# migoox/genome-downsampler

Hardware: AMD Instinct MI355X
Metric: Mreads/s selected at target coverage M=100 (higher is better)
Workload: dtype u32

## Files before the change

### genome-downsampler_amd/csrc/kernels/pass_major.inc.hip

```cpp
static constexpr int kPmPass = 8192;
__host__ __device__ inline uint32_t pm_stride_of(uint32_t n_ranges) { return (uint32_t)kPmPass + 64u * n_ranges; }
static constexpr int kPmThreads = 512;
static constexpr int kPmWaves = kPmThreads / 64;
static constexpr int kPmPassesPerWg = 4;
static constexpr size_t kPmSortLds = ((size_t)kPmPass + kPmWaves * 256 + 2 * 256 + 16 + 2 * kPmPassesPerWg * 256 + kPmWaves * 3 * 128) * sizeof(uint32_t);
static constexpr uint32_t kPmExcPerWave = 128;

#ifndef QMCP_PM_MIN_WAVES
#define QMCP_PM_MIN_WAVES 4
#endif
__global__ __launch_bounds__(kPmThreads, QMCP_PM_MIN_WAVES) void k_pm_prepare_sort(
    const uint32_t* __restrict__ starts, const uint32_t* __restrict__ ends, uint32_t n,
    const uint64_t* __restrict__ contig_read_off, const uint64_t* __restrict__ contig_pos_off, uint32_t n_contigs,
    const uint32_t* __restrict__ vbase ,
    uint32_t shift, uint32_t stride ,
    uint16_t* __restrict__ keys16, uint16_t* __restrict__ idx16,
    uint32_t* __restrict__ cnt_tab, uint32_t* __restrict__ lst_tab, uint32_t pitch ,
    uint32_t* __restrict__ stats, unsigned long long* __restrict__ zero_mask,
    uint32_t ell_reg, uint32_t* __restrict__ exc, uint32_t exc_cap, uint32_t* __restrict__ exc_cnt) {
    extern __shared__ uint32_t s_pm[];
    uint32_t* s_stage = s_pm;
    uint32_t* s_cnt = s_stage + kPmPass;
    uint32_t* s_gbase = s_cnt + kPmWaves * 256;
    uint32_t* s_pbase = s_gbase + 256;
    uint32_t* s_wave = s_pbase + 256;
    uint32_t* s_tabc = s_wave + 16;
    uint32_t* s_tabl = s_tabc + kPmPassesPerWg * 256;
    uint32_t* s_exc = s_tabl + kPmPassesPerWg * 256;
    const int lane = threadIdx.x & 63, w = threadIdx.x >> 6;
    uint32_t mn = 0xFFFFFFFFu, mx = 0, bad = 0;
    auto contig_of = [&](uint32_t i) {
        uint32_t lo = 0, hi = n_contigs;
        while (hi - lo > 1) {
            const uint32_t mid = (lo + hi) >> 1;
            if (contig_read_off[mid] <= i) lo = mid; else hi = mid;
        }
        return lo;
    };
    for (int g = 0; g < kPmPassesPerWg; ++g) {
        const uint32_t P = blockIdx.x * kPmPassesPerWg + g;
        const uint64_t base64 = (uint64_t)P * kPmPass;
        if (base64 >= n) {
            if (threadIdx.x < 256) { s_tabc[g * 256 + threadIdx.x] = 0; s_tabl[g * 256 + threadIdx.x] = 0; }
            if (ell_reg != 0u && lane == 0 && P < pitch) exc_cnt[P * kPmWaves + w] = 0;
            continue;
        }
        const uint32_t base = (uint32_t)base64;
        const uint32_t count = min((uint32_t)kPmPass, n - base);
        const uint32_t wbase = base + w * (kSortItems * 64);
        Rec rec[kSortItems];
#pragma unroll
        for (int k = 0; k < kSortItems; ++k) {
            const uint32_t i = min(wbase + k * 64 + lane, n - 1);
            rec[k].key = starts[i];
            rec[k].val = ends[i];
        }
        for (int i = threadIdx.x; i < kPmWaves * 256; i += kPmThreads) s_cnt[i] = 0;
        if (zero_mask && threadIdx.x < 128 && P * 128u + threadIdx.x < (n + 63u) / 64u) zero_mask[P * 128u + threadIdx.x] = 0ull;
        const uint32_t c_first = n_contigs > 1 ? contig_of(base) : 0u;
        const uint32_t c_last = n_contigs > 1 ? contig_of(base + count - 1) : 0u;
        uint32_t match_bits;
        {
            const uint32_t len_last = (uint32_t)(contig_pos_off[c_last + 1] - contig_pos_off[c_last]);
            const uint32_t d_lo = (vbase[c_first] >> shift) & 255u;
            const uint32_t d_hi = ((vbase[c_last] + (len_last ? len_last - 1u : 0u)) >> shift) & 255u;
            match_bits = d_hi >= d_lo ? 32u - (uint32_t)__builtin_clz((d_hi - d_lo) | 1u) : 8u;
            if (d_hi == d_lo) match_bits = 0;
        }
        uint32_t skip = 0;
        uint32_t filled = 0;
        typedef __attribute__((address_space(3))) uint32_t LdsWord;
        LdsWord* const mine = (LdsWord*)(s_exc + w * (3 * kPmExcPerWave));
        auto put_aside = [&, mine](int k, bool isx, uint32_t gs, uint32_t ge, uint32_t i) {
            const uint64_t m = __ballot(isx);
            if (m != 0ull) {
                const uint32_t slot = filled + __builtin_amdgcn_mbcnt_hi((uint32_t)(m >> 32), __builtin_amdgcn_mbcnt_lo((uint32_t)m, 0u));
                if (isx) {
                    skip |= 1u << k;
                    if (slot < kPmExcPerWave) { mine[3u * slot] = gs; mine[3u * slot + 1u] = ge; mine[3u * slot + 2u] = i; }
                    else nu_overflow_put(exc, exc_cap, stats, gs, ge, i);
                }
                filled += (uint32_t)__popcll(m);
            }
        };
        if (c_first == c_last) {
            const uint32_t p0 = (uint32_t)contig_pos_off[c_first];
            const uint32_t len = (uint32_t)contig_pos_off[c_first + 1] - p0;
            const uint32_t v0 = vbase[c_first];
            const uint32_t last = len ? len - 1u : 0u;
#pragma unroll
            for (int k = 0; k < kSortItems; ++k) {
                const uint32_t i = wbase + k * 64 + lane;
                const uint32_t s = rec[k].key, e = rec[k].val;
                bool isx = false;
                if (i < n) {
                    bad |= (s > e || e >= len) ? 1u : 0u;
                    const uint32_t span = e - s + 1;
                    mn = min(mn, span);
                    mx = max(mx, span);
                    isx = span != ell_reg;
                }
                rec[k].key = v0 + min(s, last);
                if (ell_reg != 0u) put_aside(k, isx, p0 + min(s, last), p0 + min(e, last), i);
            }
        } else {
#pragma unroll
            for (int k = 0; k < kSortItems; ++k) {
                const uint32_t i = wbase + k * 64 + lane;
                bool isx = false;
                uint32_t gs = 0, ge = 0;
                if (i < n) {
                    const uint32_t cc = contig_of(i);
                    const uint32_t p0 = (uint32_t)contig_pos_off[cc];
                    const uint32_t len = (uint32_t)contig_pos_off[cc + 1] - p0;
                    const uint32_t s = rec[k].key, e = rec[k].val;
                    bad |= (s > e || e >= len) ? 1u : 0u;
                    const uint32_t span = e - s + 1;
                    mn = min(mn, span);
                    mx = max(mx, span);
                    rec[k].key = vbase[cc] + min(s, len ? len - 1u : 0u);
                    isx = span != ell_reg;
                    gs = p0 + min(s, len ? len - 1u : 0u);
                    ge = p0 + min(e, len ? len - 1u : 0u);
                }
                if (ell_reg != 0u) put_aside(k, isx, gs, ge, i);
            }
        }
        __syncthreads();
        uint32_t rank[kSortItems];
        {
            uint32_t* const s_cnt_w = s_cnt + w * 256;
            const uint32_t bound = base + count;
            switch (match_bits) {
                case 0: part_rank_rounds<0>(rec, rank, wbase, bound, shift, lane, s_cnt_w, skip); break;
                case 1: part_rank_rounds<1>(rec, rank, wbase, bound, shift, lane, s_cnt_w, skip); break;
                case 2: part_rank_rounds<2>(rec, rank, wbase, bound, shift, lane, s_cnt_w, skip); break;
                case 3: part_rank_rounds<3>(rec, rank, wbase, bound, shift, lane, s_cnt_w, skip); break;
                case 4: part_rank_rounds<4>(rec, rank, wbase, bound, shift, lane, s_cnt_w, skip); break;
                case 5: part_rank_rounds<5>(rec, rank, wbase, bound, shift, lane, s_cnt_w, skip); break;
                case 6: part_rank_rounds<6>(rec, rank, wbase, bound, shift, lane, s_cnt_w, skip); break;
                case 7: part_rank_rounds<7>(rec, rank, wbase, bound, shift, lane, s_cnt_w, skip); break;
                default: part_rank_rounds<8>(rec, rank, wbase, bound, shift, lane, s_cnt_w, skip); break;
            }
        }
        __syncthreads();
        if (threadIdx.x < 256) {
            const uint32_t d = threadIdx.x;
            uint32_t tot = 0;
#pragma unroll
            for (int x = 0; x < kPmWaves; ++x) tot += s_cnt[x * 256 + d];
            const uint32_t ptot = (tot + 63u) & ~63u;
            const uint32_t inc = wave_incl_scan_add(tot);
            const uint32_t pinc = wave_incl_scan_add(ptot);
            if (lane == 63) { s_wave[w] = inc; s_wave[8 + w] = pinc; }
            s_gbase[d] = inc - tot;
            s_pbase[d] = pinc - ptot;
            s_tabc[g * 256 + d] = ptot;
            s_tabl[g * 256 + d] = tot << 16;
        }
        __syncthreads();
        if (threadIdx.x < 256) {
            const uint32_t d = threadIdx.x;
            uint32_t wave_base = 0, pwave_base = 0;
            for (int x = 0; x < w; ++x) { wave_base += s_wave[x]; pwave_base += s_wave[8 + x]; }
            const uint32_t tile_off = s_gbase[d] + wave_base;
            const uint32_t ptile_off = s_pbase[d] + pwave_base;
            uint32_t run = tile_off;
#pragma unroll
            for (int x = 0; x < kPmWaves; ++x) { const uint32_t cx = s_cnt[x * 256 + d]; s_cnt[x * 256 + d] = run; run += cx; }
            s_gbase[d] = tile_off;
            s_pbase[d] = ptile_off;
            s_tabl[g * 256 + d] |= ptile_off >> 6;
        }
        __syncthreads();
#pragma unroll
        for (int k = 0; k < kSortItems; ++k) {
            const uint32_t i = wbase + k * 64 + lane;
            if (i < n && !((skip >> k) & 1u)) {
                const uint32_t d = (rec[k].key >> shift) & 255u;
                const uint32_t local = (uint32_t)(w * (kSortItems * 64) + k * 64 + lane);
                s_stage[s_cnt[w * 256 + d] + rank[k]] = (rec[k].key & ((1u << shift) - 1u)) | (local << 16);
            }
        }
        __syncthreads();
        {
            const uint32_t my_d = (uint32_t)w + 8u * ((uint32_t)lane & 31u);
            const uint32_t my_tot = lane < 32 ? s_tabl[g * 256 + my_d] >> 16 : 0u;
            const uint32_t my_gb = s_gbase[my_d], my_pb = s_pbase[my_d];
            const bool upper = lane >= 32;
            const uint32_t hl = (uint32_t)lane & 31u;
            uint64_t todo = __ballot(my_tot != 0u);
            while (todo != 0ull) {
                const int l0 = __builtin_ctzll(todo);
                todo &= todo - 1ull;
                int l1 = l0;
                bool two = false;
                if (todo != 0ull) { l1 = __builtin_ctzll(todo); todo &= todo - 1ull; two = true; }
                const uint32_t cnt0 = (uint32_t)__builtin_amdgcn_readlane((int)my_tot, l0);
                const uint32_t cnt1 = two ? (uint32_t)__builtin_amdgcn_readlane((int)my_tot, l1) : 0u;
                const uint32_t cnt = upper ? cnt1 : cnt0;
                const uint32_t gb = upper ? (uint32_t)__builtin_amdgcn_readlane((int)my_gb, l1) : (uint32_t)__builtin_amdgcn_readlane((int)my_gb, l0);
                const uint32_t pb = upper ? (uint32_t)__builtin_amdgcn_readlane((int)my_pb, l1) : (uint32_t)__builtin_amdgcn_readlane((int)my_pb, l0);
                const size_t out0 = (size_t)P * stride + pb;
                const uint32_t most = max(cnt0, cnt1);
                for (uint32_t j0 = 0; j0 < most; j0 += 128u) {
                    const uint32_t j = j0 + 4u * hl;
                    if (j < cnt) {
                        const uint32_t v0 = s_stage[gb + j];
                        const uint32_t v1 = j + 1 < cnt ? s_stage[gb + j + 1] : 0u;
                        const uint32_t v2 = j + 2 < cnt ? s_stage[gb + j + 2] : 0u;
                        const uint32_t v3 = j + 3 < cnt ? s_stage[gb + j + 3] : 0u;
                        *reinterpret_cast<uint2*>(keys16 + out0 + j) = make_uint2((v0 & 0xFFFFu) | (v1 << 16), (v2 & 0xFFFFu) | (v3 << 16));
                        *reinterpret_cast<uint2*>(idx16 + out0 + j) = make_uint2((v0 >> 16) | (v1 & 0xFFFF0000u), (v2 >> 16) | (v3 & 0xFFFF0000u));
                    }
                }
            }
        }
        if (ell_reg != 0u) {
            const size_t slot0 = ((size_t)P * kPmWaves + w) * kPmExcPerWave;
            for (uint32_t r = (uint32_t)lane; r < min(filled, kPmExcPerWave); r += 64u) {
                exc[slot0 + r] = mine[3u * r];
                exc[exc_cap + slot0 + r] = mine[3u * r + 1u];
                exc[2 * (size_t)exc_cap + slot0 + r] = mine[3u * r + 2u];
            }
            if (lane == 0) {
                exc_cnt[P * kPmWaves + w] = min(filled, kPmExcPerWave);
            }
        }
        __syncthreads();
    }
    __syncthreads();
    if (threadIdx.x < 256) {
        const uint32_t P0 = blockIdx.x * kPmPassesPerWg;
        if (P0 < pitch) {
            uint4 a, b;
            a.x = s_tabc[threadIdx.x]; a.y = s_tabc[256 + threadIdx.x]; a.z = s_tabc[512 + threadIdx.x]; a.w = s_tabc[768 + threadIdx.x];
            b.x = s_tabl[threadIdx.x]; b.y = s_tabl[256 + threadIdx.x]; b.z = s_tabl[512 + threadIdx.x]; b.w = s_tabl[768 + threadIdx.x];
            *reinterpret_cast<uint4*>(cnt_tab + (size_t)threadIdx.x * pitch + P0) = a;
            *reinterpret_cast<uint4*>(lst_tab + (size_t)threadIdx.x * pitch + P0) = b;
        }
    }

    __shared__ uint32_t s_red[3][kPmWaves];
    mn = wave_min_u32(mn);
    mx = wave_max_u32(mx);
    bad = wave_max_u32(bad);
    if (lane == 0) { s_red[0][w] = mn; s_red[1][w] = mx; s_red[2][w] = bad; }
    __syncthreads();
    if (threadIdx.x == 0) {
        for (int x = 1; x < kPmWaves; ++x) { mn = min(mn, s_red[0][x]); mx = max(mx, s_red[1][x]); bad |= s_red[2][x]; }
        if (mn < __hip_atomic_load(&stats[0], __ATOMIC_RELAXED, __HIP_MEMORY_SCOPE_AGENT)) atomicMin(&stats[0], mn);
        if (mx > __hip_atomic_load(&stats[1], __ATOMIC_RELAXED, __HIP_MEMORY_SCOPE_AGENT)) atomicMax(&stats[1], mx);
        if (bad) atomicOr(&stats[2], 1u);
    }
}

static constexpr uint32_t kPmDescrY = 8;
static constexpr uint32_t kPmWorkWords = 256u * kPmDescrY * 2u;

struct PmSlot { uint32_t slot0, nv, pass; };
template <bool kVector>
__device__ __forceinline__ PmSlot pm_unpack(uint32_t dsc, bool has, uint32_t stride) {
    PmSlot s;
    s.pass = dsc >> 15;
    s.slot0 = has ? (kVector ? __umul24(s.pass, stride) : s.pass * stride) + (((dsc >> 6) & 511u) << 6) : 0u;
    s.nv = has ? (dsc & 63u) + 1u : 0u;
    return s;
}

__device__ __forceinline__ void pm_row_part(uint32_t pitch, uint32_t& P_beg, uint32_t& P_end) {
    const uint32_t per = (pitch + kPmDescrY - 1u) / kPmDescrY;
    P_beg = min(pitch, blockIdx.y * per);
    P_end = min(pitch, (blockIdx.y + 1u) * per);
}

__global__ __launch_bounds__(256) void k_pm_row_sums(const uint32_t* __restrict__ cnt_tab, const uint32_t* __restrict__ lstw,
                                                     uint32_t pitch, uint32_t* __restrict__ work) {
    __shared__ uint32_t s_red[2][4];
    const uint32_t d = blockIdx.x;
    uint32_t P_beg, P_end;
    pm_row_part(pitch, P_beg, P_end);
    uint32_t pad = 0, tru = 0;
    for (uint32_t P0 = P_beg + threadIdx.x; P0 < P_end; P0 += 4u * 256u) {
        uint32_t c[4], w[4];
#pragma unroll
        for (int u = 0; u < 4; ++u) {
            const uint32_t P = min(P0 + (uint32_t)u * 256u, P_end - 1u);
            c[u] = cnt_tab[(size_t)d * pitch + P];
            w[u] = lstw[(size_t)d * pitch + P];
        }
#pragma unroll
        for (int u = 0; u < 4; ++u)
            if (P0 + (uint32_t)u * 256u < P_end) { pad += c[u]; tru += w[u] >> 16; }
    }
    pad = wave_sum_u32(pad);
    tru = wave_sum_u32(tru);
    if ((threadIdx.x & 63u) == 0u) { s_red[0][threadIdx.x >> 6] = pad; s_red[1][threadIdx.x >> 6] = tru; }
    __syncthreads();
    if (threadIdx.x == 0) {
        uint32_t* const out = work + ((size_t)d * kPmDescrY + blockIdx.y) * 2u;
        out[0] = s_red[0][0] + s_red[0][1] + s_red[0][2] + s_red[0][3];
        out[1] = s_red[1][0] + s_red[1][1] + s_red[1][2] + s_red[1][3];
    }
}

__global__ __launch_bounds__(256) void k_pm_tables(uint32_t* tab, const uint32_t* __restrict__ lstw, uint32_t pitch,
                                                   uint32_t n_groups ,
                                                   uint32_t* __restrict__ desc, const uint32_t* __restrict__ work,
                                                   uint32_t* __restrict__ range_start,
                                                   uint32_t* __restrict__ max_load ,
                                                   uint32_t* __restrict__ clear16 ) {
    __shared__ uint32_t s_red[4], s_red2[4], s_base, s_tile[2][4][4];
    const uint32_t d = blockIdx.x, y = blockIdx.y, tid = threadIdx.x;
    const uint32_t lane = tid & 63u, wv = tid >> 6;
    const bool first = d == 0u && y == 0u;
    uint32_t rp = 0, rt = 0, before = 0;
    {
        const uint4* const src = reinterpret_cast<const uint4*>(work + (size_t)tid * kPmDescrY * 2u);
        uint4 q[kPmDescrY / 2u];
#pragma unroll
        for (uint32_t k = 0; k < kPmDescrY / 2u; ++k) q[k] = src[k];
#pragma unroll
        for (uint32_t k = 0; k < kPmDescrY / 2u; ++k) {
            if (2u * k < y) before += q[k].x;
            if (2u * k + 1u < y) before += q[k].z;
            rp += q[k].x + q[k].z;
            rt += q[k].y + q[k].w;
        }
    }
    {
        const uint32_t inc = wave_incl_scan_add(rp);
        if (lane == 63u) s_red[wv] = inc;
        __syncthreads();
        uint32_t base = 0;
        for (uint32_t x = 0; x < wv; ++x) base += s_red[x];
        if (tid == d) s_base = base + inc - rp + before;
        if (first && tid == 255u) tab[(size_t)256u * pitch] = base + inc;
        __syncthreads();
    }
    if (first) {
        if (clear16 != nullptr && tid < 16u) clear16[tid] = 0u;
        const uint32_t inc = wave_incl_scan_add(rt);
        const uint32_t mx = wave_max_u32(rt), mxp = wave_max_u32(rp);
        if (lane == 63u) s_red[wv] = inc;
        __syncthreads();
        uint32_t base = 0;
        for (uint32_t x = 0; x < wv; ++x) base += s_red[x];
        range_start[tid] = base + inc - rt;
        if (tid == 255u) range_start[256] = base + inc;
        __syncthreads();
        if (lane == 0u) { s_red[wv] = mx; s_red2[wv] = mxp; }
        __syncthreads();
        if (tid == 0) {
            max_load[0] = max(max(s_red[0], s_red[1]), max(s_red[2], s_red[3]));
            max_load[1] = max(max(s_red2[0], s_red2[1]), max(s_red2[2], s_red2[3])) >> 6;
        }
    }
    uint32_t P_beg, P_end;
    pm_row_part(pitch, P_beg, P_end);
    uint32_t carry = s_base;
    uint32_t round = 0;
    for (uint32_t P0 = P_beg; P0 < P_end; P0 += 4u * 256u, round ^= 1u) {
        uint32_t c[4], w[4], inc[4];
#pragma unroll
        for (int u = 0; u < 4; ++u) {
            const uint32_t P = P0 + (uint32_t)u * 256u + tid;
            const bool in = P < P_end;
            const size_t at = (size_t)d * pitch + min(P, P_end - 1u);
            c[u] = tab[at];
            w[u] = lstw[at];
            if (!in) { c[u] = 0u; w[u] = 0u; }
        }
#pragma unroll
        for (int u = 0; u < 4; ++u) {
            inc[u] = wave_incl_scan_add(c[u]);
            if (lane == 63u) s_tile[round][u][wv] = inc[u];
        }
        __syncthreads();
#pragma unroll
        for (int u = 0; u < 4; ++u) {
            uint32_t base = carry;
            for (uint32_t x = 0; x < wv; ++x) base += s_tile[round][u][x];
            carry += s_tile[round][u][0] + s_tile[round][u][1] + s_tile[round][u][2] + s_tile[round][u][3];
            const uint32_t P = P0 + (uint32_t)u * 256u + tid;
            if (P >= P_end) continue;
            const uint32_t t = base + inc[u] - c[u];
            tab[(size_t)d * pitch + P] = t;
            const uint32_t cnt = w[u] >> 16;
            if (cnt == 0u) continue;
            const uint32_t g = t >> 6;
            const uint32_t n_ws = (cnt + 63u) >> 6;
            for (uint32_t j = 0; j < n_ws; ++j)
                if (g + j < n_groups)
                    desc[g + j] = (P << 15) | (((w[u] & 0xFFFFu) + j) << 6) | (min(64u, cnt - 64u * j) - 1u);
        }
    }
}

__device__ __forceinline__ uint32_t pm_grid_pos0(const uint32_t* __restrict__ grid, uint32_t r) { return grid[r]; }
__device__ __forceinline__ uint32_t pm_grid_live(const uint32_t* __restrict__ grid, uint32_t r) { return grid[kPmGridRows + r]; }
__device__ __forceinline__ uint32_t pm_grid_contig(const uint32_t* __restrict__ grid, uint32_t r) { return grid[2u * kPmGridRows + r]; }

#ifndef QMCP_PM_OFFSETS_U
#define QMCP_PM_OFFSETS_U 8
#endif
__global__ __launch_bounds__(1024) void k_pm_offsets(const uint16_t* __restrict__ keys16, const uint32_t* __restrict__ desc,
                                                     const uint32_t* __restrict__ Tp, uint32_t pitch,
                                                     const uint32_t* __restrict__ range_start ,
                                                     const uint32_t* __restrict__ grid,
                                                     uint32_t shift, uint32_t stride, uint32_t ltot, uint32_t* __restrict__ boff,
                                                     uint32_t* __restrict__ empty_positions) {
    extern __shared__ uint32_t s_cnt32[];
#define PADDED(i) ((i) + ((i) >> 5))
    __shared__ uint32_t s_wsum[16], s_esum[16];
    const uint32_t range = blockIdx.x, width = 1u << shift;
    const uint32_t pos0 = pm_grid_pos0(grid, range), live = pm_grid_live(grid, range);
    const uint32_t lo_p = Tp[(size_t)range * pitch], hi_p = Tp[(size_t)(range + 1) * pitch];
    const uint32_t g0 = lo_p >> 6, n_ws = (hi_p - lo_p) >> 6;
    const uint32_t lo = range_start[range];
    for (uint32_t i = threadIdx.x; i < width; i += blockDim.x) s_cnt32[PADDED(i)] = 0;
    __syncthreads();
    const uint32_t lane = threadIdx.x & 63u, nw = blockDim.x >> 6;
    const uint32_t w = (uint32_t)__builtin_amdgcn_readfirstlane((int)(threadIdx.x >> 6));
    const uint32_t sub = lane >> 4, l16 = lane & 15u;
    constexpr int kU = QMCP_PM_OFFSETS_U;
    const uint32_t n_quads = (n_ws + 3u) >> 2;
    uint32_t dsc[kU];
    auto ask_descriptors = [&](uint32_t q0) {
#pragma unroll
        for (int u = 0; u < kU; ++u) dsc[u] = desc[g0 + min(4u * (q0 + (uint32_t)u * nw) + sub, n_ws - 1u)];
    };
    if (n_ws != 0u) ask_descriptors(w);
    for (uint32_t q0 = w; q0 < n_quads; q0 += kU * nw) {
        uint2 v[kU];
        uint32_t nv[kU];
#pragma unroll
        for (int u = 0; u < kU; ++u) {
            const PmSlot at = pm_unpack<true>(dsc[u], 4u * (q0 + (uint32_t)u * nw) + sub < n_ws, stride);
            nv[u] = at.nv;
            v[u] = *reinterpret_cast<const uint2*>(keys16 + at.slot0 + 4u * l16);
        }
        if (q0 + kU * nw < n_quads) ask_descriptors(q0 + kU * nw);
#pragma unroll
        for (int u = 0; u < kU; ++u) {
            const uint32_t e = 4u * l16;
            if (e < nv[u]) atomicAdd(&s_cnt32[PADDED(v[u].x & 0xFFFFu)], 1u);
            if (e + 1 < nv[u]) atomicAdd(&s_cnt32[PADDED(v[u].x >> 16)], 1u);
            if (e + 2 < nv[u]) atomicAdd(&s_cnt32[PADDED(v[u].y & 0xFFFFu)], 1u);
            if (e + 3 < nv[u]) atomicAdd(&s_cnt32[PADDED(v[u].y >> 16)], 1u);
        }
    }
    __syncthreads();
    const uint32_t per = width >= 1024u ? width >> 10 : 1u;
    const uint32_t firstp = threadIdx.x * per;
    uint32_t sum = 0, empties = 0;
    if (firstp < width)
        for (uint32_t qq = 0; qq < per; ++qq) {
            const uint32_t cq = s_cnt32[PADDED(firstp + qq)];
            sum += cq;
            empties += (cq == 0 && firstp + qq < live) ? 1u : 0u;
        }
    const uint32_t inc = wave_incl_scan_add(sum);
    const uint32_t wv = threadIdx.x >> 6;
    if (lane == 63) s_wsum[wv] = inc;
    if (empty_positions != nullptr) {
        empties = wave_sum_u32(empties);
        if (lane == 0) s_esum[wv] = empties;
    }
    __syncthreads();
    if (empty_positions != nullptr && threadIdx.x == 0) {
        uint32_t total = 0;
        for (uint32_t x = 0; x < nw; ++x) total += s_esum[x];
        if (total != 0) atomicAdd(empty_positions, total);
    }
    uint32_t run = lo + inc - sum;
    for (uint32_t x = 0; x < wv; ++x) run += s_wsum[x];
    if (firstp < width)
        for (uint32_t qq = 0; qq < per; ++qq) {
            const uint32_t cq = s_cnt32[PADDED(firstp + qq)];
            s_cnt32[PADDED(firstp + qq)] = run;
            run += cq;
        }
    __syncthreads();
    for (uint32_t i = threadIdx.x; i < live; i += blockDim.x) boff[pos0 + i] = s_cnt32[PADDED(i)];
    if (range == gridDim.x - 1u && threadIdx.x == 0) boff[ltot] = range_start[kPmGridRows];
#undef PADDED
}

struct EvQuota { const uint32_t* sev; const uint32_t* lastns; const uint64_t* poff; uint32_t n_contigs, ell; };

__device__ __forceinline__ uint32_t pm_settle_groups(const uint16_t* __restrict__ keys16, const uint16_t* __restrict__ idx16,
                                                     const uint32_t* __restrict__ desc, uint32_t g0, uint32_t n_ws,
                                                     uint32_t stride, const uint2* amb, uint32_t namb, uint32_t w,
                                                     uint32_t lane, unsigned long long* __restrict__ mask) {
    const uint64_t gt_mask = lane == 63 ? 0ull : ~((2ull << lane) - 1ull);
    uint32_t kept = 0;
    constexpr int kSteps = 16, kE = 2;
    constexpr uint32_t stride_k = 16;
    for (uint32_t k0 = w; k0 < namb; k0 += kE * stride_k) {
        uint32_t key[kE][kSteps], dscv[kE] , p[kE], skip[kE], c_of[kE];
#pragma unroll
        for (int x = 0; x < kE; ++x) {
            const uint32_t k = k0 + (uint32_t)x * stride_k;
            const uint2 ent = k < namb ? amb[k] : make_uint2(0u, 0u);
            c_of[x] = ent.x >> 15;
            p[x] = k < namb ? ent.x & 0x7FFFu : 0xFFFFFFFFu;
            skip[x] = ent.y;
            const uint32_t ws = 16u * c_of[x] + (lane & 15u);
            dscv[x] = ws < n_ws ? desc[g0 + ws] : 0u;
        }
#pragma unroll
        for (int x = 0; x < kE; ++x) {
#pragma unroll
            for (int t = 0; t < kSteps; ++t) {
                const uint32_t dsc = (uint32_t)__builtin_amdgcn_readlane((int)dscv[x], t);
                key[x][t] = keys16[pm_unpack<false>(dsc, 16u * c_of[x] + (uint32_t)t < n_ws, stride).slot0 + lane];
            }
        }
#pragma unroll
        for (int x = 0; x < kE; ++x) {
#pragma unroll
            for (int t = kSteps - 1; t >= 0; --t) {
                const uint32_t dsc = (uint32_t)__builtin_amdgcn_readlane((int)dscv[x], t);
                const PmSlot at = pm_unpack<false>(dsc, 16u * c_of[x] + (uint32_t)t < n_ws, stride);
                const bool member = lane < at.nv && key[x][t] == p[x];
                const uint64_t m = __ballot(member);
                if (m == 0) continue;
                const uint32_t above = (uint32_t)__popcll(m & gt_mask);
                if (member && above >= skip[x]) {
                    const uint32_t v = at.pass * (uint32_t)kPmPass + idx16[at.slot0 + lane];
                    atomicOr(&mask[v >> 6], 1ull << (v & 63u));
                }
                const uint32_t in_step = (uint32_t)__popcll(m);
                kept += in_step > skip[x] ? in_step - skip[x] : 0u;
                skip[x] = skip[x] > in_step ? skip[x] - in_step : 0u;
            }
        }
    }
    return kept;
}

__global__ __launch_bounds__(1024) void k_pm_walk(const uint16_t* __restrict__ keys16, const uint16_t* __restrict__ idx16,
                                                  const uint32_t* __restrict__ desc,
                                                  const uint32_t* __restrict__ Tp, uint32_t pitch,
                                                  const uint32_t* __restrict__ range_start ,
                                                  const uint32_t* __restrict__ grid,
                                                  uint32_t shift, uint32_t stride,
                                                  const uint32_t* __restrict__ boff, const uint32_t* __restrict__ selend,
                                                  EvQuota evq,
                                                  unsigned long long* __restrict__ mask,
                                                  uint2* __restrict__ amb_lists, int lists_by_records,
                                                  unsigned long long* __restrict__ kept_total) {
    extern __shared__ int32_t s_q[];
    __shared__ uint32_t s_namb, s_kept;
    __shared__ uint32_t s_ring[16][128];
    const uint32_t range = blockIdx.x, width = 1u << shift;
    const uint32_t pos0 = pm_grid_pos0(grid, range), live = pm_grid_live(grid, range);
    const uint32_t tid = threadIdx.x, nthreads = blockDim.x;
    const uint32_t lane = tid & 63u;
    const uint32_t w = (uint32_t)__builtin_amdgcn_readfirstlane((int)(tid >> 6));
    const uint32_t lo_p = Tp[(size_t)range * pitch];
    const uint32_t hi_p = Tp[(size_t)(range + 1) * pitch];
    if (lo_p >= hi_p) return;
    const uint32_t g0 = lo_p >> 6, n_ws = (hi_p - lo_p) >> 6;
    const uint32_t n_chunks = (n_ws + 15u) >> 4;
    const uint32_t lo_true = range_start[range];
    uint2* const amb = amb_lists + (lists_by_records ? (size_t)lo_true : (size_t)range * width);
    if (evq.sev != nullptr) {
        const uint32_t c_range = pm_grid_contig(grid, range);
        for (uint32_t i0 = tid; i0 < live; i0 += 8 * nthreads) {
            uint32_t src[8], back[8];
#pragma unroll
            for (int u = 0; u < 8; ++u) {
                const uint32_t p = pos0 + min(i0 + u * nthreads, live - 1);
                uint32_t c_lo = c_range, c_hi = c_range + 1u;
                if (c_range == kPmNoContig) { c_lo = 0; c_hi = evq.n_contigs; }
                while (c_hi - c_lo > 1) {
                    const uint32_t mid = (c_lo + c_hi) >> 1;
                    if ((uint32_t)evq.poff[mid] <= p) c_lo = mid; else c_hi = mid;
                }
                const uint32_t base = (uint32_t)evq.poff[c_lo];
                const uint32_t k = (p - base) / evq.ell;
                src[u] = p;
                back[u] = k - evq.lastns[(size_t)(base / (4u * evq.ell) + c_lo) * 4u + k];
            }
#pragma unroll
            for (int u = 0; u < 8; ++u) src[u] = evq.sev[src[u] - back[u] * evq.ell];
#pragma unroll
            for (int u = 0; u < 8; ++u)
                if (i0 + u * nthreads < live) s_q[i0 + u * nthreads] = (int32_t)src[u];
        }
    } else
    for (uint32_t i0 = tid; i0 < live; i0 += 8 * nthreads) {
        uint32_t a[8], b[8];
#pragma unroll
        for (int u = 0; u < 8; ++u) {
            const uint32_t i = min(i0 + u * nthreads, live - 1);
            a[u] = selend[pos0 + i];
            b[u] = boff[pos0 + i];
        }
#pragma unroll
        for (int u = 0; u < 8; ++u)
            if (i0 + u * nthreads < live) s_q[i0 + u * nthreads] = (int32_t)(a[u] - b[u]);
    }
    if (tid == 0) { s_namb = 0; s_kept = 0; }
    __syncthreads();

#define QMCP_PM_RING "v96", "v97", "v98", "v99", "v100", "v101", "v102", "v103", "v104", "v105", "v106", "v107", "v108", "v109", "v110", "v111", "v112", "v113", "v114", "v115", "v116", "v117", "v118", "v119"
#define QMCP_PM_KEYREG(k) "v" QMCP_PM_STR(QMCP_PM_CAT(QMCP_PM_KEY_, k))
#define QMCP_PM_DSCREG(k) "v" QMCP_PM_STR(QMCP_PM_CAT(QMCP_PM_DSC_, k))
#define QMCP_PM_IDXREG(k) "v" QMCP_PM_STR(QMCP_PM_CAT(QMCP_PM_IDX_, k))
#define QMCP_PM_STR(x) QMCP_PM_STR2(x)
#define QMCP_PM_STR2(x) #x
#define QMCP_PM_CAT(a, b) QMCP_PM_CAT2(a, b)
#define QMCP_PM_CAT2(a, b) a##b
#define QMCP_PM_KEY_0 96
#define QMCP_PM_KEY_1 97
#define QMCP_PM_KEY_2 98
#define QMCP_PM_KEY_3 99
#define QMCP_PM_KEY_4 100
#define QMCP_PM_KEY_5 101
#define QMCP_PM_KEY_6 102
#define QMCP_PM_KEY_7 103
#define QMCP_PM_DSC_0 104
#define QMCP_PM_DSC_1 105
#define QMCP_PM_DSC_2 106
#define QMCP_PM_DSC_3 107
#define QMCP_PM_DSC_4 108
#define QMCP_PM_DSC_5 109
#define QMCP_PM_DSC_6 110
#define QMCP_PM_DSC_7 111
#define QMCP_PM_IDX_0 112
#define QMCP_PM_IDX_1 113
#define QMCP_PM_IDX_2 114
#define QMCP_PM_IDX_3 115
#define QMCP_PM_IDX_4 116
#define QMCP_PM_IDX_5 117
#define QMCP_PM_IDX_6 118
#define QMCP_PM_IDX_7 119
    static_assert(kRankDepth == 8, "the ring registers are named for eight slots");
    struct Slot { uint32_t slot0, nv, read0; bool has; };
    auto desc_offset = [&](uint32_t c) -> uint32_t {
        return (g0 + min(16u * c + w, n_ws - 1u)) * 4u;
    };
    auto slot_of = [&](uint32_t dsc, uint32_t c) -> Slot {
        const bool has = 16u * c + w < n_ws;
        const PmSlot at = pm_unpack<true>(dsc, has, stride);
        Slot s;
        s.slot0 = at.slot0;
        s.nv = at.nv;
        s.read0 = at.pass * (uint32_t)kPmPass;
        s.has = has;
        return s;
    };
    uint32_t kept = 0;
    uint32_t cur = 0, flushed = 0;
    uint32_t* const ring = s_ring[w];
#define QMCP_PM_STEP(K, KF)                                                                                                   \
    {                                                                                                                         \
        const uint32_t c = c0 + (uint32_t)(K);                                                                                \
        uint32_t key, dsc, idx;                                                                                               \
        asm volatile("s_waitcnt vmcnt(19)\n\tv_mov_b32 %0, " QMCP_PM_KEYREG(K) "\n\tv_mov_b32 %1, " QMCP_PM_DSCREG(K)          \
                     "\n\tv_mov_b32 %2, " QMCP_PM_IDXREG(K)                                                                   \
                     : "=v"(key), "=v"(dsc), "=v"(idx) : : QMCP_PM_RING, "memory");                                                      \
        const Slot at = S[K];                                                                                                 \
        const bool valid = lane < at.nv;                                                                                      \
        int32_t old = 0;                                                                                                      \
        if (valid) old = atomicSub(&s_q[key], 1);                                         \
        S[KF] = slot_of(dsc, c + 7u);                                                                                         \
        asm volatile("global_load_ushort " QMCP_PM_KEYREG(KF) ", %0, %1\n\tglobal_load_ushort " QMCP_PM_IDXREG(KF) ", %0, %2"   \
                     "\n\tglobal_load_dword " QMCP_PM_DSCREG(K) ", %3, %4"                                                    \
                     : : "v"((S[KF].slot0 + lane) * 2u), "s"(keys16), "s"(idx16), "v"(desc_offset(c + 15u)), "s"(desc)        \
                     : QMCP_PM_RING, "memory");                                                                               \
        __syncthreads();                                                                                                      \
        int32_t aft = 0;                                                                                                      \
        if (valid) aft = s_q[key];                                                                                            \
        const bool keep = valid && old > 0 && aft >= 0;                                                                       \
        if (valid && old == 1 && aft < 0) {                                                                                   \
            const uint32_t k = atomicAdd(&s_namb, 1u);                                                                        \
            amb[k] = make_uint2((c << 15) | key, (uint32_t)(-aft));                                 \
        }                                                                                                                     \
        __syncthreads();                                               \
        if (at.has) {                                                    \
            const uint64_t kb = __ballot(keep);                                                                               \
            const uint32_t cw = (uint32_t)__popcll(kb);                                                                       \
            if (keep) ring[(cur + __builtin_amdgcn_mbcnt_hi((uint32_t)(kb >> 32), __builtin_amdgcn_mbcnt_lo((uint32_t)kb, 0u))) & 127u] = at.read0 + idx; \
            cur += cw;                                                                                                        \
            if (cur - flushed >= 64u) {                                                                          \
                const uint32_t v = ring[(flushed + lane) & 127u];                                                             \
                atomicOr(&mask[v >> 6], 1ull << (v & 63u));                                                                   \
                flushed += 64u;                                                                                               \
            }                                                                                                                 \
        }                                                                                                                     \
    }
    Slot S[kRankDepth];
    {
        uint32_t d0[kRankDepth - 1];
#pragma unroll
        for (int k = 0; k < kRankDepth - 1; ++k) d0[k] = desc[desc_offset((uint32_t)k) / 4u];
#pragma unroll
        for (int k = 0; k < kRankDepth - 1; ++k) S[k] = slot_of(d0[k], (uint32_t)k);
        S[kRankDepth - 1] = Slot{0u, 0u, 0u, false};
#define QMCP_PM_ASK_KEYS(K) asm volatile("global_load_ushort " QMCP_PM_KEYREG(K) ", %0, %1\n\tglobal_load_ushort " QMCP_PM_IDXREG(K) ", %0, %2" : : "v"((S[K].slot0 + lane) * 2u), "s"(keys16), "s"(idx16) : QMCP_PM_RING, "memory");
#define QMCP_PM_ASK_DSC(K) asm volatile("global_load_dword " QMCP_PM_DSCREG(K) ", %0, %1" : : "v"(desc_offset(7u + (uint32_t)(K))), "s"(desc) : QMCP_PM_RING, "memory");
        QMCP_PM_ASK_KEYS(0) QMCP_PM_ASK_KEYS(1) QMCP_PM_ASK_KEYS(2) QMCP_PM_ASK_KEYS(3) QMCP_PM_ASK_KEYS(4) QMCP_PM_ASK_KEYS(5) QMCP_PM_ASK_KEYS(6)
        QMCP_PM_ASK_DSC(0) QMCP_PM_ASK_DSC(1) QMCP_PM_ASK_DSC(2) QMCP_PM_ASK_DSC(3) QMCP_PM_ASK_DSC(4) QMCP_PM_ASK_DSC(5) QMCP_PM_ASK_DSC(6) QMCP_PM_ASK_DSC(7)
        asm volatile("s_waitcnt vmcnt(0)" : : : QMCP_PM_RING, "memory");
#undef QMCP_PM_ASK_KEYS
#undef QMCP_PM_ASK_DSC
    }
    for (uint32_t c0 = 0; c0 < n_chunks; c0 += kRankDepth) {
        QMCP_PM_STEP(0, 7) QMCP_PM_STEP(1, 0) QMCP_PM_STEP(2, 1) QMCP_PM_STEP(3, 2)
        QMCP_PM_STEP(4, 3) QMCP_PM_STEP(5, 4) QMCP_PM_STEP(6, 5) QMCP_PM_STEP(7, 6)
    }
#undef QMCP_PM_STEP
    asm volatile("s_waitcnt vmcnt(0)" : : : QMCP_PM_RING, "memory");
    if (lane < cur - flushed) {
        const uint32_t v = ring[(flushed + lane) & 127u];
        atomicOr(&mask[v >> 6], 1ull << (v & 63u));
    }
    kept = cur;
    __syncthreads();
    kept += pm_settle_groups(keys16, idx16, desc, g0, n_ws, stride, amb, s_namb, w, lane, mask);
    if (lane == 0 && kept) atomicAdd(&s_kept, kept);
    __syncthreads();
    if (tid == 0 && s_kept) atomicAdd(kept_total, (unsigned long long)s_kept);
}

uint32_t pm_pitch(uint32_t n) { return part_pass_pitch(n); }
uint32_t pm_pass() { return (uint32_t)kPmPass; }
uint32_t pm_stride(uint32_t n_ranges) { return pm_stride_of(n_ranges); }
size_t pm_slots(uint32_t n, uint32_t n_ranges) { return (size_t)pm_pitch(n) * pm_stride(n_ranges); }
uint32_t pm_work_words() { return kPmWorkWords; }
uint32_t pm_exc_slots(uint32_t n) { return pm_pitch(n) * kPmWaves * kPmExcPerWave + kNuOverflow; }
bool pm_rank_scratch_by_records(uint32_t shift, uint32_t n_ranges, uint32_t n) { return (size_t)n < ((size_t)n_ranges << shift); }
size_t pm_rank_scratch_bytes(uint32_t shift, uint32_t n_ranges, uint32_t n) {
    const size_t by_pos = (size_t)n_ranges << shift;
    return (by_pos < (size_t)n ? by_pos : (size_t)n) * sizeof(uint2) + 64;
}
void launch_pm_prepare_sort(hipStream_t st, const uint32_t* starts, const uint32_t* ends, uint32_t n,
                            const uint64_t* d_roff, const uint64_t* d_poff, uint32_t n_contigs, uint32_t shift,
                            uint32_t n_ranges, const uint32_t* d_grid,
                            uint16_t* keys16, uint16_t* idx16, uint32_t* cnt_tab, uint32_t* lst_tab,
                            uint32_t* stats, unsigned long long* zero_mask, uint32_t ell_reg, uint32_t* exc,
                            uint32_t exc_cap, uint32_t* exc_cnt) {
    const uint32_t pitch = pm_pitch(n);
    if (pitch == 0) return;
    (void)hipFuncSetAttribute((const void*)k_pm_prepare_sort, hipFuncAttributeMaxDynamicSharedMemorySize, (int)kPmSortLds);
    hipLaunchKernelGGL(k_pm_prepare_sort, dim3(pitch / kPmPassesPerWg), dim3(kPmThreads), kPmSortLds, st, starts, ends, n,
                       d_roff, d_poff, n_contigs, d_grid + 3u * kPmGridRows, shift, pm_stride(n_ranges), keys16, idx16,
                       cnt_tab, lst_tab, pitch, stats, zero_mask, exc != nullptr ? ell_reg : 0u, exc, exc_cap, exc_cnt);
    if (exc != nullptr && ell_reg != 0u)
        hipLaunchKernelGGL(k_nu_count_groups, dim3(32), dim3(256), 0, st, exc_cnt, pitch * kPmWaves, stats);
}
void launch_pm_row_sums(hipStream_t st, const uint32_t* cnt_tab, const uint32_t* lstw, uint32_t n, uint32_t* work) {
    const uint32_t pitch = pm_pitch(n);
    if (pitch == 0) return;
    hipLaunchKernelGGL(k_pm_row_sums, dim3(256, kPmDescrY), dim3(256), 0, st, cnt_tab, lstw, pitch, work);
}
void launch_pm_tables(hipStream_t st, uint32_t* tab, const uint32_t* lstw, uint32_t n, uint32_t n_ranges,
                      uint32_t* desc, const uint32_t* work, uint32_t* range_start, uint32_t* max_load, uint32_t* clear16) {
    const uint32_t pitch = pm_pitch(n);
    if (pitch == 0) return;
    const uint32_t s64 = pm_stride(n_ranges) / 64u;
    hipLaunchKernelGGL(k_pm_tables, dim3(256, kPmDescrY), dim3(256), 0, st, tab, lstw, pitch, pitch * s64, desc, work,
                       range_start, max_load, clear16);
}
void launch_pm_offsets(hipStream_t st, const uint16_t* keys16, const uint32_t* desc, const uint32_t* Tp, uint32_t n,
                       const uint32_t* range_start, uint32_t shift, uint32_t n_ranges, const uint32_t* d_grid, uint32_t ltot,
                       uint32_t* boff, uint32_t* empty_positions) {
    const size_t width = (size_t)1 << shift;
    const size_t lds = (width + width / 32 + 1) * sizeof(uint32_t);
    (void)hipFuncSetAttribute((const void*)k_pm_offsets, hipFuncAttributeMaxDynamicSharedMemorySize, (int)lds);
    hipLaunchKernelGGL(k_pm_offsets, dim3(n_ranges), dim3(1024), lds, st, keys16, desc, Tp, pm_pitch(n), range_start, d_grid,
                       shift, pm_stride(n_ranges), ltot, boff, empty_positions);
}
void launch_pm_walk(hipStream_t st, const uint16_t* keys16, const uint16_t* idx16, const uint32_t* desc, const uint32_t* Tp,
                    uint32_t n, const uint32_t* range_start, uint32_t shift, uint32_t n_ranges, const uint32_t* d_grid,
                    const uint32_t* boff, const uint32_t* selend, unsigned long long* mask, unsigned long long* kept_total, void* scratch,
                    bool scratch_by_records, const uint32_t* ev_sev, const uint32_t* ev_lastns,
                    const uint64_t* d_poff, uint32_t n_contigs, uint32_t ell) {
    const EvQuota evq{ev_sev, ev_lastns, d_poff, n_contigs, ell};
    const size_t lds = (((size_t)1 << shift) + 1) * sizeof(uint32_t);
    (void)hipFuncSetAttribute((const void*)k_pm_walk, hipFuncAttributeMaxDynamicSharedMemorySize, (int)lds);
    hipLaunchKernelGGL(k_pm_walk, dim3(n_ranges), dim3(1024), lds, st, keys16, idx16, desc, Tp, pm_pitch(n), range_start, d_grid, shift,
                       pm_stride(n_ranges), boff, selend, evq, mask, (uint2*)scratch, scratch_by_records ? 1 : 0,
                       kept_total);
}
```

### genome-downsampler_amd/csrc/qmcp_kernels.hip

```cpp
#include <hip/hip_runtime.h>
#include <stdint.h>

#include <type_traits>

#include "qmcp_kernels.h"
#include "target_table.h"

namespace qmcp {

static constexpr int kWave = 64;
static constexpr uint32_t kInf = 0x40000000u;

#include "kernels/wave_primitives.inc.hip"
#include "kernels/prepare_scan.inc.hip"
#include "kernels/radix_sort.inc.hip"
#include "kernels/ranked_route.inc.hip"
#include "kernels/bucket_offsets.inc.hip"
#include "kernels/sweep_uniform.inc.hip"
#include "kernels/sweep_segments.inc.hip"
#include "kernels/sweep_uniform_pipelines.inc.hip"
#include "kernels/sweep_uniform_events.inc.hip"
#include "kernels/sweep_mixed.inc.hip"
#include "kernels/mark_and_next_rows.inc.hip"
#include "kernels/launchers.inc.hip"
#include "kernels/pass_major.inc.hip"
#include "kernels/near_uniform.inc.hip"
#include "kernels/by_contig.inc.hip"
#include "kernels/ladder.inc.hip"
#include "kernels/amplicon_by_contig.inc.hip"
#include "kernels/quality_cells.inc.hip"
#include "kernels/targets.inc.hip"
#include "kernels/depth_report.inc.hip"
#include "kernels/depth_track.inc.hip"
#include "kernels/stratified.inc.hip"
#include "kernels/dedup.inc.hip"
#include "kernels/profile.inc.hip"
#include "kernels/pairs.inc.hip"
#include "kernels/templates.inc.hip"
#include "kernels/templates_profile.inc.hip"
#include "kernels/fragments.inc.hip"
#include "kernels/ceiling.inc.hip"
#include "kernels/proportional.inc.hip"
#include "kernels/budget.inc.hip"
#include "kernels/mean_depth.inc.hip"
#include "kernels/thresholds.inc.hip"
#include "kernels/replicates.inc.hip"

}
```

Baseline: 126,500.

## Use blocked per-lane layout with LDS lane-count ranking in pass-major sort

When the pass's digit range is narrow (at most 32 digits) and the input pointers are 16-byte aligned with no regular-length exception list, each lane now owns 16 consecutive records. It loads them with vector quad loads and ranks them using packed 16-bit per-lane counters in LDS plus a wave-wide scan, replacing the multi-round match-based ranking. The per-pass contig and digit-range computation is also hoisted one pass ahead so its scalar loads overlap with the current pass. This adds a second ranking path and new LDS ordering fences, and the blocked path is skipped when ell_reg is nonzero.

```diff
diff --git a/genome-downsampler_amd/csrc/kernels/pass_major.inc.hip b/genome-downsampler_amd/csrc/kernels/pass_major.inc.hip
--- a/genome-downsampler_amd/csrc/kernels/pass_major.inc.hip
+++ b/genome-downsampler_amd/csrc/kernels/pass_major.inc.hip
@@ -37,6 +37,29 @@
         }
         return lo;
     };
+    struct PassForm { uint32_t c_first, c_last, match_bits, d_lo, d_hi; };
+    auto form_of = [&](uint32_t base, uint32_t count) {
+        PassForm f;
+        f.c_first = n_contigs > 1 ? contig_of(base) : 0u;
+        f.c_last = n_contigs > 1 ? contig_of(base + count - 1) : 0u;
+        const uint32_t len_last = (uint32_t)(contig_pos_off[f.c_last + 1] - contig_pos_off[f.c_last]);
+        f.d_lo = (vbase[f.c_first] >> shift) & 255u;
+        f.d_hi = ((vbase[f.c_last] + (len_last ? len_last - 1u : 0u)) >> shift) & 255u;
+        f.match_bits = f.d_hi >= f.d_lo ? 32u - (uint32_t)__builtin_clz((f.d_hi - f.d_lo) | 1u) : 8u;
+        if (f.d_hi == f.d_lo) f.match_bits = 0;
+        f.c_first = (uint32_t)__builtin_amdgcn_readfirstlane((int)f.c_first);
+        f.c_last = (uint32_t)__builtin_amdgcn_readfirstlane((int)f.c_last);
+        f.d_lo = (uint32_t)__builtin_amdgcn_readfirstlane((int)f.d_lo);
+        f.d_hi = (uint32_t)__builtin_amdgcn_readfirstlane((int)f.d_hi);
+        f.match_bits = (uint32_t)__builtin_amdgcn_readfirstlane((int)f.match_bits);
+        return f;
+    };
+    const bool lane_form_ok = ell_reg == 0u && (((uintptr_t)starts | (uintptr_t)ends) & 15u) == 0u;
+    PassForm next_form = {0u, 0u, 0u, 0u, 0u};
+    {
+        const uint64_t base0 = (uint64_t)blockIdx.x * kPmPassesPerWg * kPmPass;
+        if (base0 < n) next_form = form_of((uint32_t)base0, min((uint32_t)kPmPass, n - (uint32_t)base0));
+    }
     for (int g = 0; g < kPmPassesPerWg; ++g) {
         const uint32_t P = blockIdx.x * kPmPassesPerWg + g;
         const uint64_t base64 = (uint64_t)P * kPmPass;
@@ -48,25 +71,33 @@
         const uint32_t base = (uint32_t)base64;
         const uint32_t count = min((uint32_t)kPmPass, n - base);
         const uint32_t wbase = base + w * (kSortItems * 64);
+        const PassForm form = next_form;
+        const uint32_t c_first = form.c_first, c_last = form.c_last, match_bits = form.match_bits;
+        const bool blocked = lane_form_ok && match_bits <= kPmLaneFormBits;
+        const uint32_t lane0 = wbase + (blocked ? 16u * (uint32_t)lane : (uint32_t)lane);
+        const uint32_t kstep = blocked ? 1u : 64u;
         Rec rec[kSortItems];
-#pragma unroll
-        for (int k = 0; k < kSortItems; ++k) {
-            const uint32_t i = min(wbase + k * 64 + lane, n - 1);
-            rec[k].key = starts[i];
-            rec[k].val = ends[i];
+        if (blocked && count == (uint32_t)kPmPass) {
+            const PmQuad* const s4 = reinterpret_cast<const PmQuad*>(starts + lane0);
+            const PmQuad* const e4 = reinterpret_cast<const PmQuad*>(ends + lane0);
+#pragma unroll
+            for (int q = 0; q < kSortItems / 4; ++q) {
+                const PmQuad s = s4[q], e = e4[q];
+                rec[4 * q].key = s.x; rec[4 * q + 1].key = s.y; rec[4 * q + 2].key = s.z; rec[4 * q + 3].key = s.w;
+                rec[4 * q].val = e.x; rec[4 * q + 1].val = e.y; rec[4 * q + 2].val = e.z; rec[4 * q + 3].val = e.w;
+            }
+        } else {
+#pragma unroll
+            for (int k = 0; k < kSortItems; ++k) {
+                const uint32_t i = min(lane0 + k * kstep, n - 1);
+                rec[k].key = starts[i];
+                rec[k].val = ends[i];
+            }
         }
         for (int i = threadIdx.x; i < kPmWaves * 256; i += kPmThreads) s_cnt[i] = 0;
         if (zero_mask && threadIdx.x < 128 && P * 128u + threadIdx.x < (n + 63u) / 64u) zero_mask[P * 128u + threadIdx.x] = 0ull;
-        const uint32_t c_first = n_contigs > 1 ? contig_of(base) : 0u;
-        const uint32_t c_last = n_contigs > 1 ? contig_of(base + count - 1) : 0u;
-        uint32_t match_bits;
-        {
-            const uint32_t len_last = (uint32_t)(contig_pos_off[c_last + 1] - contig_pos_off[c_last]);
-            const uint32_t d_lo = (vbase[c_first] >> shift) & 255u;
-            const uint32_t d_hi = ((vbase[c_last] + (len_last ? len_last - 1u : 0u)) >> shift) & 255u;
-            match_bits = d_hi >= d_lo ? 32u - (uint32_t)__builtin_clz((d_hi - d_lo) | 1u) : 8u;
-            if (d_hi == d_lo) match_bits = 0;
-        }
+        if (g + 1 < kPmPassesPerWg && base64 + kPmPass < n)
+            next_form = form_of(base + kPmPass, min((uint32_t)kPmPass, n - base - (uint32_t)kPmPass));
         uint32_t skip = 0;
         uint32_t filled = 0;
         typedef __attribute__((address_space(3))) uint32_t LdsWord;
@@ -90,7 +121,7 @@
             const uint32_t last = len ? len - 1u : 0u;
 #pragma unroll
             for (int k = 0; k < kSortItems; ++k) {
-                const uint32_t i = wbase + k * 64 + lane;
+                const uint32_t i = lane0 + k * kstep;
                 const uint32_t s = rec[k].key, e = rec[k].val;
                 bool isx = false;
                 if (i < n) {
@@ -106,7 +137,7 @@
         } else {
 #pragma unroll
             for (int k = 0; k < kSortItems; ++k) {
-                const uint32_t i = wbase + k * 64 + lane;
+                const uint32_t i = lane0 + k * kstep;
                 bool isx = false;
                 uint32_t gs = 0, ge = 0;
                 if (i < n) {
@@ -131,7 +162,12 @@
         {
             uint32_t* const s_cnt_w = s_cnt + w * 256;
             const uint32_t bound = base + count;
-            switch (match_bits) {
+            if (blocked) {
+                PmLdsWord* const s_w = (PmLdsWord*)(s_stage + w * (kSortItems * 64));
+                const uint32_t n_pairs = (form.d_hi - form.d_lo) / 2u + 1u;
+                if (count == (uint32_t)kPmPass) pm_rank_lane_counts<true>(rec, rank, lane0, bound, shift, form.d_lo, n_pairs, lane, s_w, s_cnt_w);
+                else pm_rank_lane_counts<false>(rec, rank, lane0, bound, shift, form.d_lo, n_pairs, lane, s_w, s_cnt_w);
+            } else switch (match_bits) {
                 case 0: part_rank_rounds<0>(rec, rank, wbase, bound, shift, lane, s_cnt_w, skip); break;
                 case 1: part_rank_rounds<1>(rec, rank, wbase, bound, shift, lane, s_cnt_w, skip); break;
                 case 2: part_rank_rounds<2>(rec, rank, wbase, bound, shift, lane, s_cnt_w, skip); break;
@@ -175,10 +211,10 @@
         __syncthreads();
 #pragma unroll
         for (int k = 0; k < kSortItems; ++k) {
-            const uint32_t i = wbase + k * 64 + lane;
+            const uint32_t i = lane0 + k * kstep;
             if (i < n && !((skip >> k) & 1u)) {
                 const uint32_t d = (rec[k].key >> shift) & 255u;
-                const uint32_t local = (uint32_t)(w * (kSortItems * 64) + k * 64 + lane);
+                const uint32_t local = i - base;
                 s_stage[s_cnt[w * 256 + d] + rank[k]] = (rec[k].key & ((1u << shift) - 1u)) | (local << 16);
             }
         }
diff --git a/genome-downsampler_amd/csrc/kernels/pm_lane_rank.inc.hip b/genome-downsampler_amd/csrc/kernels/pm_lane_rank.inc.hip
--- /dev/null
+++ b/genome-downsampler_amd/csrc/kernels/pm_lane_rank.inc.hip
@@ -0,0 +1,60 @@
+typedef __attribute__((address_space(3))) uint32_t PmLdsWord;
+typedef uint32_t PmQuad __attribute__((ext_vector_type(4)));
+typedef __attribute__((address_space(3))) PmQuad PmLdsQuad;
+
+static constexpr uint32_t kPmLaneFormBits = 5;
+
+__device__ __forceinline__ void pm_wave_lds_order() {
+    __builtin_amdgcn_fence(__ATOMIC_ACQ_REL, "wavefront");
+    __builtin_amdgcn_wave_barrier();
+}
+
+template <bool kFull>
+__device__ __forceinline__ void pm_rank_lane_counts(const Rec (&rec)[kSortItems], uint32_t (&rank)[kSortItems],
+                                                    uint32_t first, uint32_t bound, uint32_t shift, uint32_t d_lo,
+                                                    uint32_t n_pairs , int lane,
+                                                    PmLdsWord* __restrict__ s_w ,
+                                                    uint32_t* __restrict__ s_cnt_w ) {
+    static_assert(kSortItems == 16, "a lane's sixteen records: 64 lanes x 16 pair words fill the wave's share of the stage");
+#pragma unroll
+    for (uint32_t g = 0; g < 4; ++g)
+        if (4u * g < n_pairs) ((PmLdsQuad*)s_w)[g * 64u + (uint32_t)lane] = (PmQuad)(0u);
+    pm_wave_lds_order();
+#pragma unroll
+    for (int j = 0; j < kSortItems; ++j) {
+        const uint32_t rel = ((rec[j].key >> shift) & 255u) - d_lo;
+        const uint32_t field = (rel & 1u) << 4;
+        const uint32_t at = ((rel >> 1) & 15u) * 64u + (uint32_t)lane;
+        const uint32_t one = kFull || first + (uint32_t)j < bound ? 1u << field : 0u;
+        rank[j] = __hip_atomic_fetch_add(s_w + at, one, __ATOMIC_RELAXED, __HIP_MEMORY_SCOPE_WAVEFRONT);
+    }
+    pm_wave_lds_order();
+#pragma unroll
+    for (uint32_t g = 0; g < 4; ++g) {
+        if (4u * g < n_pairs) {
+            uint32_t v[4];
+#pragma unroll
+            for (uint32_t t = 0; t < 4; ++t) v[t] = s_w[(4u * g + t) * 64u + (uint32_t)lane];
+#pragma unroll
+            for (uint32_t t = 0; t < 4; ++t) v[t] = wave_incl_scan_add(v[t]);
+#pragma unroll
+            for (uint32_t t = 0; t < 4; ++t) s_w[(4u * g + t) * 64u + (((uint32_t)lane + 1u) & 63u)] = v[t];
+        }
+    }
+    pm_wave_lds_order();
+    if (lane < 32) {
+        const uint32_t r = (uint32_t)lane;
+        if (r < 2u * n_pairs && d_lo + r < 256u) s_cnt_w[d_lo + r] = (s_w[(r >> 1) * 64u] >> ((r & 1u) << 4)) & 0xFFFFu;
+    }
+    pm_wave_lds_order();
+    if ((uint32_t)lane < n_pairs) s_w[(uint32_t)lane * 64u] = 0u;
+    pm_wave_lds_order();
+#pragma unroll
+    for (int j = 0; j < kSortItems; ++j) {
+        const uint32_t rel = ((rec[j].key >> shift) & 255u) - d_lo;
+        const uint32_t field = (rel & 1u) << 4;
+        const uint32_t at = ((rel >> 1) & 15u) * 64u + (uint32_t)lane;
+        rank[j] = ((rank[j] + s_w[at]) >> field) & 0xFFFFu;
+    }
+    pm_wave_lds_order();
+}
diff --git a/genome-downsampler_amd/csrc/qmcp_kernels.hip b/genome-downsampler_amd/csrc/qmcp_kernels.hip
--- a/genome-downsampler_amd/csrc/qmcp_kernels.hip
+++ b/genome-downsampler_amd/csrc/qmcp_kernels.hip
@@ -23,6 +23,7 @@
 #include "kernels/sweep_mixed.inc.hip"
 #include "kernels/mark_and_next_rows.inc.hip"
 #include "kernels/launchers.inc.hip"
+#include "kernels/pm_lane_rank.inc.hip"
 #include "kernels/pass_major.inc.hip"
 #include "kernels/near_uniform.inc.hip"
 #include "kernels/by_contig.inc.hip"
```

Measured after the change: 132,300 (median of 6 runs). +4.6%, better.
